# rizar/attention-lvcsr

Hardware: AMD Instinct MI355X
Metric: encoder+attention+decoder training frames/sec (whole node) (higher is better)
Workload: dtype f32; 1 GPU; wsj_base: B=16 utterances x T=800 frames x F=40 fbank per GPU, L=100 labels; 256x256x256x256 BiGRU subsample [1, 1, 2, 2], content_and_conv attention, 256-unit GRU decoder; global_batch=16, per_gpu_batch=16, ragged=False, parallelism=dp1, optimizer=clip100+adadelta+maxnorm1, hip_graph=True, priming_steps=2, encoder_kernels=persistent clusters, full=False

## Files before the change

attention-lvcsr_amd/csrc/gemm.hip:

```cpp
#include "common.h"
#include "lvsr_hip.h"
#include "graph_cache.h"
#include <algorithm>
#include <vector>

#define BM 64
#define BN 64
#define BK 16
#define LDS_LD (BM + 4)

struct GemmArgs {
    const float* A; const float* B; float* C; const float* bias;
    int M, N, K, lda, ldb, ldc, transA, transB;
    float alpha, beta;
    int ksplit;
    int kchunk;
    float* part;
    int batch;
    long long sA, sB, sC;
};

__global__ __launch_bounds__(256) void lvsr_sgemm_kernel(GemmArgs g) {
    __shared__ float As[BK][LDS_LD];
    __shared__ float Bs[BK][LDS_LD];
// ... 577 lines not shown
#define COPY_MANY_MAX 32
struct CopyPack { lvsr_copy_desc d[COPY_MANY_MAX]; int n; };
__global__ __launch_bounds__(256) void lvsr_copy2d_many_kernel(CopyPack pk) {
    const lvsr_copy_desc& d = pk.d[blockIdx.y];
    const bool vec = ((d.cols | d.lds | d.ldd) & 3) == 0 && ((((size_t)d.src) | ((size_t)d.dst)) & 15) == 0;
    if (d.rows == 1) {
        for (int c = blockIdx.x * 256 + threadIdx.x; c < d.cols; c += gridDim.x * 256)
            d.dst[c] = d.beta != 0.f ? d.src[c] + d.beta * d.dst[c] : d.src[c];
        return;
    }
    for (int r = blockIdx.x; r < d.rows; r += gridDim.x) {
        const float* s = d.src + (size_t)r * d.lds;
        float* o = d.dst + (size_t)r * d.ldd;
        if (d.beta != 0.f) {
            for (int c = threadIdx.x; c < d.cols; c += 256) o[c] = s[c] + d.beta * o[c];
        } else if (vec) {
            for (int c = threadIdx.x * 4; c < d.cols; c += 1024) *(float4*)(o + c) = *(const float4*)(s + c);
        } else {
            for (int c = threadIdx.x; c < d.cols; c += 256) o[c] = s[c];
        }
    }
}

__global__ __launch_bounds__(256) void lvsr_transpose_kernel(const float* in, int rows, int cols, float* out) {
    __shared__ float tile[32][33];
    const int tx = threadIdx.x & 31, ty = threadIdx.x >> 5;
    const int r0 = blockIdx.y * 32, c0 = blockIdx.x * 32;
    for (int j = ty; j < 32; j += 8) {
        const int r = r0 + j, c = c0 + tx;
        tile[j][tx] = (r < rows && c < cols) ? in[(size_t)r * cols + c] : 0.f;
    }
    __syncthreads();
    for (int j = ty; j < 32; j += 8) {
        const int c = c0 + j, r = r0 + tx;
        if (r < rows && c < cols) out[(size_t)c * rows + r] = tile[tx][j];
    }
}

__global__ __launch_bounds__(256) void lvsr_pack_b_kernel(const float* W, int ldw, int K, int N, int trans, float* P,
                                                          int Kw, int NQ, long long total) {
    for (long long idx = (long long)blockIdx.x * 256 + threadIdx.x; idx < total; idx += (long long)gridDim.x * 256) {
        const int r = (int)(idx & 3), lane = (int)((idx >> 2) & 63);
        const long long g = idx >> 8;
        const int q = (int)(g % NQ), wave = (int)((g / NQ) & 3), tile = (int)(g / NQ / 4);
        const int k = wave * Kw + (lane >> 4) * (Kw >> 2) + 4 * q + r, col = tile * 16 + (lane & 15);
        float v = 0.f;
        if (k < K && col < N) v = trans ? W[(size_t)col * ldw + k] : W[(size_t)k * ldw + col];
        P[idx] = v;
    }
}

static bool operands_aligned(const float* A, int lda, const float* B, int ldb) {
    return (lda & 3) == 0 && (ldb & 3) == 0 && (((size_t)A) & 15) == 0 && (((size_t)B) & 15) == 0;
}

static int colsum_split(int M, int N, bool have_ws, long long ws_bytes) {
    if (!have_ws || M < 512) return 1;
    const int nx = (N + 63) / 64;
    int S = (M + 255) / 256;
    const int want = (1024 + nx - 1) / nx;
    if (S > want) S = want;
    while (S > 1 && (long long)S * N * 4 > ws_bytes) --S;
    return S;
}

extern "C" {

static int sgemm_launch(void* stream, int transA, int transB, int M, int N, int K, float alpha, const float* A, int lda,
                        const float* B, int ldb, float beta, float* C, int ldc, const float* bias, float* ws,
                        long long ws_bytes, int batch, long long sA, long long sB, long long sC) {
    LVSR_REQUIRE(M >= 0 && N >= 0 && K >= 0 && batch >= 1, "lvsr_sgemm: negative dimension");
    if (M == 0 || N == 0) return LVSR_OK;
    GemmArgs g;
    g.batch = batch; g.sA = sA; g.sB = sB; g.sC = sC;
    if (batch > 1) ws = nullptr;
    g.A = A; g.B = B; g.C = C; g.bias = bias;
    g.M = M; g.N = N; g.K = K; g.lda = lda; g.ldb = ldb; g.ldc = ldc; g.transA = transA; g.transB = transB;
    g.alpha = alpha; g.beta = beta; g.ksplit = 1; g.kchunk = 0; g.part = nullptr;
    const bool big = (M >= 96 && N >= 96) || (min(M, N) >= 32 && max(M, N) >= 256 && K >= 2048);
    int tm = big ? GM : BM, tn = big ? GN : BN;
    const int tk = big ? GK : BK;
    int tiles = ((M + tm - 1) / tm) * ((N + tn - 1) / tn);
    const int mid_max = lvsr_knob(LVSR_KNOB_GEMM_MID_TILES) > 0 ? lvsr_knob(LVSR_KNOB_GEMM_MID_TILES) : 2048;
    const bool mid = big && batch == 1 && (tiles < 256 || (tiles < mid_max && K <= 2048));
    if (mid) { tm = 64; tn = 64; tiles = ((M + 63) / 64) * ((N + 63) / 64); }
    g.kchunk = ((K + tk - 1) / tk) * tk;
    if (g.kchunk == 0) g.kchunk = tk;
    const int slots = mid ? 1024 : 512;
    if (ws && 2 * tiles <= slots && K >= 1024) {
        int want = (slots + tiles - 1) / tiles;
        int maxk = K / 256;
        if (want > maxk) want = maxk;
        long long need = (long long)want * M * N * 4;
        while (want > 1 && need > ws_bytes) { --want; need = (long long)want * M * N * 4; }
        if (want > 1) {
            int chunk = (K + want - 1) / want;
            chunk = ((chunk + tk - 1) / tk) * tk;
            g.ksplit = (K + chunk - 1) / chunk;
            g.kchunk = chunk;
            g.part = ws;
        }
    }
    dim3 grid((N + tn - 1) / tn, (M + tm - 1) / tm, batch > 1 ? batch : g.ksplit);
    hipStream_t st = (hipStream_t)stream;
    if (!big) {
        hipLaunchKernelGGL(lvsr_sgemm_kernel, grid, dim3(256), 0, st, g);
    } else {
        const bool fast = operands_aligned(A, lda, B, ldb) && (batch == 1 || ((sA & 3) == 0 && (sB & 3) == 0));
        lvsr_dispatch<0, 1, 2, 3, 4, 5, 6, 7>((transA ? 4 : 0) | (transB ? 2 : 0) | (fast ? 1 : 0), [&](auto v) {
            constexpr bool TA = (decltype(v)::value & 4) != 0, TB = (decltype(v)::value & 2) != 0, FAST = (decltype(v)::value & 1) != 0;
            if (mid) hipLaunchKernelGGL((lvsr_sgemm64_kernel<TA, TB, FAST>), grid, dim3(256), 0, st, g);
            else hipLaunchKernelGGL((lvsr_sgemm128_kernel<TA, TB, FAST>), grid, dim3(256), 0, st, g);
        });
    }
    if (g.ksplit > 1) {
        int nb = (int)(((size_t)M * N + 255) / 256);
        if (nb > 2048) nb = 2048;
        hipLaunchKernelGGL(lvsr_sgemm_splitk_reduce, dim3(nb), dim3(256), 0, st, g);
    }
    return lvsr_check_launch("lvsr_sgemm");
}

int lvsr_sgemm(void* stream, int transA, int transB, int M, int N, int K, float alpha, const float* A, int lda,
               const float* B, int ldb, float beta, float* C, int ldc, const float* bias, float* ws,
               long long ws_bytes) {
    return sgemm_launch(stream, transA, transB, M, N, K, alpha, A, lda, B, ldb, beta, C, ldc, bias, ws, ws_bytes, 1, 0, 0, 0);
}

int lvsr_sgemm_batched(void* stream, int transA, int transB, int M, int N, int K, float alpha, const float* A, int lda,
                       long long strideA, const float* B, int ldb, long long strideB, float beta, float* C, int ldc,
                       long long strideC, int batch) {
    LVSR_REQUIRE(batch >= 0, "lvsr_sgemm_batched: negative batch");
    if (batch == 0) return LVSR_OK;
    return sgemm_launch(stream, transA, transB, M, N, K, alpha, A, lda, B, ldb, beta, C, ldc, nullptr, nullptr, 0, batch,
                        strideA, strideB, strideC);
}

static bool group_aligned(const lvsr_gemm_desc& s) { return operands_aligned(s.A, s.lda, s.B, s.ldb); }
static void group_cut(const lvsr_gemm_desc* s, int n, long long ws_bytes, int* ksplit, int* kchunk) {
    int target = 1024;
    if (ws_bytes > 0) {
        for (;; target += 512) {
            long long need = 0;
            bool splits = false;
            for (int i = 0; i < n; ++i) {
                const int want = (s[i].K + target - 1) / target;
                if (want > 1) { need += ((long long)want * s[i].M * s[i].N + 3) / 4 * 4; splits = true; }
            }
            if (!splits || need * 4 <= ws_bytes) break;
        }
    }
    for (int i = 0; i < n; ++i) {
        const int want = ws_bytes > 0 ? (s[i].K + target - 1) / target : 1;
        int chunk = (s[i].K + want - 1) / want;
        chunk = ((chunk + GK - 1) / GK) * GK;
        kchunk[i] = chunk;
        ksplit[i] = (s[i].K + chunk - 1) / chunk;
    }
}
static void group_order(const lvsr_gemm_desc* s, const int* kchunk, int n, int* order) {
    for (int i = 0; i < n; ++i) order[i] = i;
    auto cost = [&](int i) { return (kchunk[i] < s[i].K ? kchunk[i] : s[i].K) * (group_aligned(s[i]) ? 1 : 2); };
    std::stable_sort(order, order + n, [&](int a, int b) { return cost(a) > cost(b); });
}

int lvsr_sgemm_tn_grouped_plan(const lvsr_gemm_desc* descs, int n, long long ws_bytes, int* ksplit, int* kchunk) {
    LVSR_REQUIRE(n >= 0 && (n == 0 || (descs && ksplit && kchunk)), "lvsr_sgemm_tn_grouped_plan: bad arguments");
// ... 152 lines not shown
```

attention-lvcsr_amd/csrc/optimizer.hip:

```cpp
#include "common.h"
#include "lvsr_hip.h"
#include <string.h>

typedef lvsr_opt_args Opt;

__device__ __forceinline__ float blk_sum256(float v, float* red) {
    v = wave_sum(v);
    __syncthreads();
    if ((threadIdx.x & 63) == 0) red[threadIdx.x >> 6] = v;
    __syncthreads();
    return (red[0] + red[1]) + (red[2] + red[3]);
}

__global__ __launch_bounds__(256) void opt_sqnorm_kernel(Opt o) {
    __shared__ float red[4];
    float s = 0.f;
    for (long long i = (long long)blockIdx.x * 256 + threadIdx.x; i < o.n; i += (long long)gridDim.x * 256) {
        const float g = o.grad[i] * o.grad_scale;
        s += g * g;
    }
    s = blk_sum256(s, red);
    if (threadIdx.x == 0) o.scratch[2 + blockIdx.x] = s;
}

__global__ __launch_bounds__(256) void opt_norm_kernel(Opt o, int nparts) {
    __shared__ float red[4];
    float s = 0.f;
    for (int i = threadIdx.x; i < nparts; i += 256) s += o.scratch[2 + i];
    s = blk_sum256(s, red);
    if (threadIdx.x == 0) {
        const float norm = sqrtf(s);
        const bool skip = o.guard && o.guard[0] != 0.f;
        o.scratch[3] = skip ? 1.f : 0.f;
        double* cs = skip ? nullptr : o.clip_state;
        const float thr = cs ? (float)cs[0] : o.clip_threshold;
        o.scratch[0] = norm;
        o.scratch[1] = (thr > 0.f && !(norm < thr)) ? thr / norm : 1.f;
        float burn = 0.f;
        if (cs) {
            if (cs[4] > 0.0) { burn = 1.f; cs[4] -= 1.0; }
            if (o.adaptive_clipping && norm > 0.f && norm - norm == 0.f) {
                const double d = (double)o.adaptive_decay, init = (double)o.clip_threshold, bp = (double)o.adaptive_burnin;
                const double ln = log((double)norm);
                cs[3] += 1.0;
                cs[1] = d * cs[1] + (1.0 - d) * ln;
                cs[2] = d * cs[2] + (1.0 - d) * ln * ln;
                const double var = cs[2] - cs[1] * cs[1];
                double t = exp(cs[1] + sqrt(var > 0.0 ? var : 0.0));
                const double conf = (cs[3] < bp ? cs[3] : bp) / bp;
                t = conf * t + (1.0 - conf) * init;
                cs[0] = t < 5.0 * init ? t : 5.0 * init;
            }
        }
        o.scratch[2] = burn;
    }
}

__global__ __launch_bounds__(256) void opt_rules_kernel(Opt o) {
    if (o.scratch[3] != 0.f) return;
    const float mult = o.scratch[1];
    if (blockIdx.x == 0)
        for (int sgi = threadIdx.x; sgi < o.nseg; sgi += 256) o.segflag[sgi] = 0;
    for (long long i = (long long)blockIdx.x * 256 + threadIdx.x; i < o.n; i += (long long)gridDim.x * 256) {
        float s = o.grad[i] * o.grad_scale * mult;
        if (o.use_momentum) {
            s = o.learning_rate * s;
            s = o.momentum * o.velocity[i] + s;
            o.velocity[i] = s;
        }
        if (o.use_adadelta) {
            const float ms = o.decay_rate * o.ms_step[i] + (1.f - o.decay_rate) * s * s;
            const float dx = sqrtf(o.ms_dx[i] + o.epsilon) / sqrtf(ms + o.epsilon) * s;
            o.ms_step[i] = ms;
            o.ms_dx[i] = o.decay_rate * o.ms_dx[i] + (1.f - o.decay_rate) * dx * dx;
            s = dx;
        }
        o.step[i] = s;
    }
}

#define MAXNORM_GROUPS 16
__global__ __launch_bounds__(64 * MAXNORM_GROUPS) void opt_maxnorm_kernel(Opt o) {
    __shared__ float red[MAXNORM_GROUPS][64];
    const long long* seg = o.segments + 4 * (long long)blockIdx.y;
    const long long off = seg[0], rows = seg[1], cols = seg[2], flags = seg[3];
    if (!(flags & 1) || o.scratch[3] != 0.f) return;
    const long long j = (long long)blockIdx.x * 64 + (threadIdx.x & 63);
    if ((long long)blockIdx.x * 64 >= cols) return;
    const int g = threadIdx.x >> 6;
    float s = 0.f;
    if (j < cols)
        for (long long r = g; r < rows; r += MAXNORM_GROUPS) {
            const float v = o.param[off + r * cols + j] - o.step[off + r * cols + j];
            s += v * v;
        }
    red[g][threadIdx.x & 63] = s;
    __syncthreads();
    const int c = threadIdx.x & 63;
    float tot = 0.f;
#pragma unroll
    for (int gg = 0; gg < MAXNORM_GROUPS; ++gg) tot += red[gg][c];
    const float norm = sqrtf(tot);
    if (j < cols && norm > o.max_norm) {
        const float k = o.max_norm / norm;
        for (long long r = g; r < rows; r += MAXNORM_GROUPS) {
            const long long x = off + r * cols + j;
            o.step[x] = o.param[x] - k * (o.param[x] - o.step[x]);
        }
    }
}

__global__ __launch_bounds__(256) void opt_finite_kernel(Opt o) {
    __shared__ float red[4];
    const long long* seg = o.segments + 4 * (long long)blockIdx.y;
    const long long off = seg[0], n = seg[1] * seg[2];
    if (o.scratch[3] != 0.f) return;
    float s = 0.f;
    for (long long i = (long long)blockIdx.x * 256 + threadIdx.x; i < n; i += (long long)gridDim.x * 256) s += o.step[off + i];
    s = blk_sum256(s, red);
    if (threadIdx.x == 0 && (s != s || s - s != 0.f)) o.segflag[blockIdx.y] = 1;
}

__global__ __launch_bounds__(256) void opt_apply_kernel(Opt o) {
    const long long* seg = o.segments + 4 * (long long)blockIdx.y;
    const long long off = seg[0], n = seg[1] * seg[2];
    const int bad = o.remove_not_finite ? o.segflag[blockIdx.y] : 0;
    if (o.scratch[3] != 0.f) return;
    if (o.clip_state && o.scratch[2] != 0.f) return;
    for (long long i = (long long)blockIdx.x * 256 + threadIdx.x; i < n; i += (long long)gridDim.x * 256) {
        const float p = o.param[off + i];
        const float s = bad ? (1.f - o.nonfinite_scaler) * p : o.step[off + i];
        o.param[off + i] = p - s;
    }
}

struct GuardPack { const int* w[64]; int n; };
__global__ void guard_collect_kernel(GuardPack pk, float* out) {
    if (threadIdx.x == 0) {
        int bad = 0;
        for (int i = 0; i < pk.n; ++i)
            if (pk.w[i] && __hip_atomic_load(pk.w[i], __ATOMIC_RELAXED, __HIP_MEMORY_SCOPE_AGENT) != 0) ++bad;
        out[0] = (float)bad;
    }
}

extern "C" int lvsr_guard_collect(void* stream, const int* const* words, int n, float* out) {
    LVSR_REQUIRE(n >= 0 && n <= 64 && out && (n == 0 || words), "lvsr_guard_collect: at most 64 words");
    GuardPack pk;
    pk.n = n;
    for (int i = 0; i < 64; ++i) pk.w[i] = i < n ? words[i] : nullptr;
    hipLaunchKernelGGL(guard_collect_kernel, dim3(1), dim3(64), 0, (hipStream_t)stream, pk, out);
    return lvsr_check_launch("lvsr_guard_collect");
}

extern "C" int lvsr_opt_step(void* stream, const lvsr_opt_args* args) {
    LVSR_REQUIRE(args != nullptr, "lvsr_opt_step: null args");
    Opt o;
    memcpy(&o, args, sizeof(o));
    LVSR_REQUIRE(o.n > 0 && o.nseg > 0 && o.param && o.grad && o.step && o.segments && o.scratch && o.segflag,
                 "lvsr_opt_step: missing buffers");
    LVSR_REQUIRE(!o.use_momentum || o.velocity, "lvsr_opt_step: momentum needs a velocity buffer");
    LVSR_REQUIRE(!o.use_adadelta || (o.ms_step && o.ms_dx), "lvsr_opt_step: AdaDelta needs its two accumulators");
    LVSR_REQUIRE(!o.adaptive_clipping || (o.clip_state && o.clip_threshold > 0.f && o.adaptive_burnin > 0),
                 "lvsr_opt_step: adaptive clipping needs clip_state, an initial threshold and a burn-in period");
    hipStream_t s = (hipStream_t)stream;
    const int nparts = 256;
    int nb = (int)((o.n + 255) / 256);
    if (nb > 2048) nb = 2048;
    hipLaunchKernelGGL(opt_sqnorm_kernel, dim3(nparts), dim3(256), 0, s, o);
    hipLaunchKernelGGL(opt_norm_kernel, dim3(1), dim3(256), 0, s, o, nparts);
    hipLaunchKernelGGL(opt_rules_kernel, dim3(nb), dim3(256), 0, s, o);
    if (o.max_norm > 0.f)
        hipLaunchKernelGGL(opt_maxnorm_kernel, dim3((o.max_cols + 63) / 64, o.nseg), dim3(64 * MAXNORM_GROUPS), 0, s, o);
    if (o.remove_not_finite)
        hipLaunchKernelGGL(opt_finite_kernel, dim3(16, o.nseg), dim3(256), 0, s, o);
    hipLaunchKernelGGL(opt_apply_kernel, dim3(16, o.nseg), dim3(256), 0, s, o);
    return lvsr_check_launch("lvsr_opt_step");
}
```

attention-lvcsr_amd/lvsr_amd/bricks/__init__.py:

```python
import contextlib

import torch


class SpeechBottom(object):
    ACT = {"identity": 0, "rectifier": 2, "tanh": 3}

    def __init__(self, dims, store, lib, workspace):
        self.d, self.store, self.lib, self.ws = dims, store, lib, workspace
        self._saved = None

    def apply(self, recordings, save_for_backward=True):
        d, p, lib, ws = self.d, self.store.p, self.lib, self.ws
        if not d.bottom_dims:
            return recordings
        T, B = int(recordings.shape[0]), int(recordings.shape[1])
        x = recordings.contiguous().view(T * B, d.F)
        saved = []
        for j, o in enumerate(d.bottom_dims):
            z = ws.get("bottom%d.z" % j, (T * B, o))
            lib.sgemm(x, p["/recognizer/bottom/bottom/linear_%d.W" % j], z, bias=p["/recognizer/bottom/bottom/linear_%d.b" % j])
            a = ws.get("bottom%d.a" % j, (T * B, o))
            lib.call("lvsr_act_fwd", lib.stream_for(a), self.ACT[d.bottom_act], native_ptr(z), o, T * B, o, native_ptr(a), o)
            saved.append((x, z))
# ... 10 lines not shown
        da = d_out.contiguous().view(-1, d.bottom_dims[-1])
        n = int(da.shape[0])
        for j in reversed(range(len(d.bottom_dims))):
            x, z = self._saved[j]
            o = d.bottom_dims[j]
            dz = ws.get("bottom%d.dz" % j, (n, o))
            lib.call("lvsr_act_bwd", lib.stream_for(dz), self.ACT[d.bottom_act], native_ptr(z), o, native_ptr(da), o, n, o,
                     native_ptr(dz), o)
            W = "/recognizer/bottom/bottom/linear_%d.W" % j
            lib.sgemm(x, dz, g[W], transA=True, ws=gws)
            lib.colsum(dz, g["/recognizer/bottom/bottom/linear_%d.b" % j], ws=gws)
            if j > 0:
                dx = ws.get("bottom%d.dx" % j, (n, int(x.shape[1])))
                lib.sgemm(dz, p[W], dx, transB=True)
                da = dx


def native_ptr(t):
    from ..native import ptr
    return ptr(t)


class Encoder(object):
    PERSIST_MAX_ROWS = 2

    PASS_ROWS = 64

    def __init__(self, dims, store, lib, workspace, use_graph=True, use_persistent=None, pfx="enc"):
        can = not lib.is_emulator or lib.emulates_concurrency()
        self.persist_auto = use_persistent is None
        self.use_persistent = can and (not lib.is_emulator if use_persistent is None else bool(use_persistent))
        self.d = dims
        self.store = store
        self.lib = lib
        self.ws = workspace
        self.use_graph = use_graph
        self.pfx = pfx
        self._passes = []
        self.force_passes = False
        self._pass_cols = None
        self._saved = None
        self._packs = {}
        self._cats = {}
        self._pack_cache = {}
        self.overlap = False
        self._side = None
        self._side_pending = False

    def _n(self, i, what):
        return "%s%d.%s" % (self.pfx, i, what)

    def _names(self, i, direction):
        base = "/recognizer/encoder/bidir%d/%s" % (i, direction)
        return dict(Wi=base + "/fork/fork_inputs.W", bi=base + "/fork/fork_inputs.b",
                    Wg=base + "/fork/fork_gate_inputs.W", bg=base + "/fork/fork_gate_inputs.b",
                    Whh=base + "/gatedrecurrent.state_to_state", Whg=base + "/gatedrecurrent.state_to_gates",
                    h0=base + "/gatedrecurrent.initial_state")

    def _packed(self, i):
        if self._packs.get("version") != self.store.version or self.lib.capturing:
            p, lib, ws = self.store.p, self.lib, self.ws
            packs, jobs = dict(version=self.store.version), []
            for li in range(self.d.n_layers):
                H = self.d.Hs[li]
                ent = dict(Whh=[], Whg=[], WhhT=[], WhgT=[])
                for di, direction in enumerate(("forward", "backward")):
                    n = self._names(li, direction)
                    for key, W, trans in (("Whh", p[n["Whh"]], False), ("Whg", p[n["Whg"]], False), ("WhhT", p[n["Whh"]], True)):
                        K, N = (W.shape[1], W.shape[0]) if trans else (W.shape[0], W.shape[1])
                        buf = ws.get("enc%d.%d.%s_p" % (li, di, key), (lib.pack_size(K, N),))
                        jobs.append((W, buf, trans))
                        ent[key].append(buf)
                    sz = lib.pack_size(H, H)
                    buf = ws.get("enc%d.%d.WhgT_p" % (li, di), (2 * sz,))
                    Wg = p[n["Whg"]]
                    jobs.append((Wg[:, :H], buf[:sz], True))
                    jobs.append((Wg[:, H:], buf[sz:], True))
                    ent["WhgT"].append(buf)
                packs[li] = ent
            lib.pack_many(jobs, use_graph=self.use_graph, cache=self._pack_cache)
            self._packs = packs
        return self._packs[i]

    def _fork_cat(self, i):
        ent = self._cats.get(i)
        if ent is None or ent["version"] != self.store.version or self.lib.capturing:
            p, ws = self.store.p, self.ws
            H, I = self.d.Hs[i], self.d.layer_input_dim(i)
            W = ws.get("enc%d.Wcat" % i, (I, 6 * H))
            b = ws.get("enc%d.bcat" % i, (6 * H,))
            pairs = []
            for di, direction in enumerate(("forward", "backward")):
                n = self._names(i, direction)
                o = di * 3 * H
                pairs += [(p[n["Wi"]], W[:, o: o + H]), (p[n["Wg"]], W[:, o + H: o + 3 * H]),
                          (p[n["bi"]], b[o: o + H]), (p[n["bg"]], b[o + H: o + 3 * H])]
            self.lib.copy_many(pairs)
            ent = dict(version=self.store.version, W=W, b=b)
            self._cats[i] = ent
        return ent["W"], ent["b"]

    @contextlib.contextmanager
    def _side_stream(self):
        if not self.overlap or self.lib.is_emulator or not torch.cuda.is_available():
            yield self.ws.get("gemm_ws", (1 << 22,))
            return
        cur = torch.cuda.current_stream()
        if self._side is None:
            self._side = torch.cuda.Stream(cur.device)
        self._side.wait_stream(cur)
        with torch.cuda.stream(self._side):
            yield self.ws.get("gemm_ws.side", (1 << 22,))
        self._side_pending = True

    def join_side_stream(self):
        if self._side is not None and self._side_pending:
            torch.cuda.current_stream().wait_stream(self._side)
            self._side_pending = False

    def _sync_ws(self, i, B, H):
        if not self.use_persistent:
            return None
        nbytes = int(self.lib._lvsr_bigru_persist_ws_bytes(int(B), int(H)))
        if nbytes <= 0:
            return None
        if self.persist_auto and int(self.lib._lvsr_bigru_persist_rows(int(B), int(H))) > self.PERSIST_MAX_ROWS:
            return None
        return self.ws.get(self._n(i, "sync"), ((nbytes + 3) // 4,), torch.int32)

    def check_persistent(self):
        for k, t in self.ws._bufs.items():
            if k[0].startswith("enc") and k[0].endswith(".sync") and int(t[0]) != 0:
                t[:64].zero_()
                raise RuntimeError("persistent BiGRU kernel aborted (a work-group of the cluster was not scheduled); results since "
                                   "the last check are invalid")

    def _pass_columns(self, B):
        if B <= self.PASS_ROWS or self.pfx != "enc":
            return None
        if not self.force_passes:
            if not (self.persist_auto and self.use_persistent):
                return None
            H = max(self.d.Hs)
            if int(self.lib._lvsr_bigru_persist_ws_bytes(int(B), int(H))) > 0 and \
                    int(self.lib._lvsr_bigru_persist_rows(int(B), int(H))) <= self.PERSIST_MAX_ROWS:
                return None
        n = (B + self.PASS_ROWS - 1) // self.PASS_ROWS
        per = (B + n - 1) // n
        return [(lo, min(B, lo + per)) for lo in range(0, B, per)]

    def _pass_encoder(self, k):
        while len(self._passes) <= k:
            child = Encoder(self.d, self.store, self.lib, self.ws, use_graph=self.use_graph, use_persistent=None,
                            pfx="enc.p%d_" % len(self._passes))
            child._cats = self._cats
            self._passes.append(child)
        return self._passes[k]

    @staticmethod
    def _cols2d(t, lo, hi):
        T, B = int(t.shape[0]), int(t.shape[1])
        F = int(t.numel() // max(1, T * B))
        return t.view(T, B * F)[:, lo * F: hi * F]

    def _apply_in_passes(self, cols, input_, mask, save_for_backward):
        d, lib, ws = self.d, self.lib, self.ws
        T, B = int(input_.shape[0]), int(input_.shape[1])
        F = int(input_.shape[2])
        x = input_.contiguous()
        m = None if mask is None else mask.contiguous()
        enc = msk = None
        for k, (lo, hi) in enumerate(cols):
            child = self._pass_encoder(k)
            xk = ws.get(child.pfx + ".x", (T, hi - lo, F))
            pairs = [(self._cols2d(x, lo, hi), xk.view(T, (hi - lo) * F))]
            mk = None
            if m is not None:
                mk = ws.get(child.pfx + ".m", (T, hi - lo))
                pairs.append((self._cols2d(m, lo, hi), mk))
            lib.copy_many(pairs)
            ek, emk = child.apply(xk, mk, save_for_backward=save_for_backward)
            if enc is None:
                Te, E = int(ek.shape[0]), int(ek.shape[2])
                enc = ws.get("enc.passes.encoded", (Te, B, E))
                msk = ws.get("enc.passes.mask", (Te, B))
            lib.copy_many([(ek.view(Te, (hi - lo) * E), self._cols2d(enc, lo, hi)), (emk, self._cols2d(msk, lo, hi))])
        if save_for_backward:
            self._pass_cols = cols
            self._saved = None
        return enc, msk

    def _encoder_gradient_range(self):
        offs = self.store.offsets
        mine = [(o, n) for k, (o, n) in offs.items() if k.startswith("/recognizer/encoder/")]
        lo, hi = min(o for o, n in mine), max(o + (n + 3) // 4 * 4 for o, n in mine)
        assert all(k.startswith("/recognizer/encoder/") == (lo <= o < hi) for k, (o, n) in offs.items()), "encoder parameters are not one range"
        return lo, min(hi, self.store.grad.numel()) - lo

    def _backward_in_passes(self, cols, d_encoded, need_input_grad, group=None):
        d, lib, ws = self.d, self.lib, self.ws
        dy = d_encoded.contiguous()
        Te, B, E = int(dy.shape[0]), int(dy.shape[1]), int(dy.shape[2])
        first, count = self._encoder_gradient_range()
        genc = self.store.grad[first: first + count]
        acc = ws.get("enc.passes.gacc", (count,))
        dx = None
        if group is None:
            group = lib.group()
        for k, (lo, hi) in enumerate(cols):
            child = self._passes[k]
            dk = ws.get(child.pfx + ".dy", (Te, hi - lo, E))
            lib.copy_many([(self._cols2d(dy, lo, hi), dk.view(Te, (hi - lo) * E))])
            dxk = child.backward(dk, need_input_grad=need_input_grad, group=group)
            group.flush(ws.get("gemm_ws.grouped", (1 << 26,)))
            child.finish_backward()
            if need_input_grad:
                if dx is None:
                    dx = ws.get("enc.passes.dx", (int(dxk.shape[0]), B, int(dxk.shape[2])))
                lib.copy_many([(dxk.view(int(dxk.shape[0]), -1), self._cols2d(dx, lo, hi))])
            if k + 1 < len(cols):
                lib.copy_many([(genc, acc, 0.0 if k == 0 else 1.0)])
            else:
                lib.copy_many([(acc, genc, 1.0)])
        self._scatter = []
        return dx

    def apply(self, input_, mask=None, save_for_backward=True):
        d, p, lib, ws = self.d, self.store.p, self.lib, self.ws
        T, B = int(input_.shape[0]), int(input_.shape[1])
        cols = self._pass_columns(B)
        if cols is not None:
            return self._apply_in_passes(cols, input_, mask, save_for_backward)
        if save_for_backward:
            self._pass_cols = None
        x = input_.contiguous()
        m = None if mask is None else mask.contiguous()
        saved = []
        gemm_ws = ws.get("gemm_ws", (1 << 22,))
        for i, (H, s) in enumerate(zip(d.Hs, d.subsample)):
            I = d.layer_input_dim(i)
            Ts = (T + s - 1) // s
            xg = ws.get(self._n(i, "xg"), (T, B, 6 * H))
            y = ws.get(self._n(i, "y"), (T, B, 2 * H))
            ysub = y if s == 1 else ws.get(self._n(i, "ysub"), (Ts, B, 2 * H))
            u = ws.get(self._n(i, "u"), (T, B, 2 * H))
            r = ws.get(self._n(i, "r"), (T, B, 2 * H))
            c = ws.get(self._n(i, "c"), (T, B, 2 * H))
            rh = ws.get(self._n(i, "rh"), (T, B, 2 * H))
            x2, xg2 = x.view(T * B, I), xg.view(T * B, 6 * H)
            sync = self._sync_ws(i, B, H)
            pk = self._packed(i) if sync is None else None
            Wcat, bcat = self._fork_cat(i)
            lib.sgemm(x2, Wcat, xg2, bias=bcat)
            h0s = [p[self._names(i, direction)["h0"]] for direction in ("forward", "backward")]
            if sync is not None:
                nf, nb = self._names(i, "forward"), self._names(i, "backward")
                Whh, Whg = [p[nf["Whh"]], p[nb["Whh"]]], [p[nf["Whg"]], p[nb["Whg"]]]
            else:
                Whh, Whg = [pk["Whh"][0], pk["Whh"][1]], [pk["Whg"][0], pk["Whg"][1]]
            lib.run("lvsr_bigru_fwd", "lvsr_bigru_fwd_args", y, self.use_graph and sync is None, xg=xg, mask=m, Whh_p=Whh, Whg_p=Whg, h0=h0s,
                    y=y, ysub=(ysub if s > 1 else None), u=u, r=r, c=c, rh=rh, sub=s, T=T, B=B, H=H,
                    persistent=int(sync is not None), sync_ws=sync)
            saved.append(dict(x=x, mask=m, T=T, y=y, u=u, r=r, c=c, rh=rh))
            x = ysub
            if m is not None and s > 1:
                mm = ws.get(self._n(i, "msub"), (Ts, B))
                mm.copy_(m[::s])
                m = mm
            T = Ts
        if m is None:
            m = ws.get(self.pfx + ".ones_mask", (T, B))
            m.fill_(1.0)
        if save_for_backward:
            self._saved = saved
        return x, m

    def backward(self, d_encoded, need_input_grad=False, group=None):
        d, p, g, lib, ws = self.d, self.store.p, self.store.g, self.lib, self.ws
        if self._pass_cols is not None:
            return self._backward_in_passes(self._pass_cols, d_encoded, need_input_grad, group)
        assert self._saved is not None, "apply() must run first"
        gemm_ws = ws.get("gemm_ws", (1 << 22,))
        self._scatter = []
        dy = d_encoded.contiguous()
        B = int(dy.shape[1])
        for i in reversed(range(d.n_layers)):
            H, s, I = d.Hs[i], d.subsample[i], d.layer_input_dim(i)
            sv = self._saved[i]
            T = sv["T"]
            dxg = ws.get(self._n(i, "dxg"), (T, B, 6 * H))
            Bp = (B + 15) // 16 * 16
            dh_ws = ws.get(self._n(i, "dh"), (12 * Bp * H,))
            nf, nb = self._names(i, "forward"), self._names(i, "backward")
            sync = self._sync_ws(i, B, H)
            pk = self._packed(i) if sync is None else None
            if sync is not None:
                WhhT, WhgT = [p[nf["Whh"]], p[nb["Whh"]]], [p[nf["Whg"]], p[nb["Whg"]]]
            else:
                WhhT, WhgT = [pk["WhhT"][0], pk["WhhT"][1]], [pk["WhgT"][0], pk["WhgT"][1]]
            lib.run("lvsr_bigru_bwd", "lvsr_bigru_bwd_args", dxg, self.use_graph and sync is None, mask=sv["mask"], y=sv["y"],
                    u=sv["u"], r=sv["r"], c=sv["c"], WhhT_p=WhhT, WhgT_p=WhgT, h0=[p[nf["h0"]], p[nb["h0"]]], dy=dy,
                    dxg=dxg, dh_ws=dh_ws, dh0=[g[nf["h0"]], g[nb["h0"]]], sub=s, T=T, B=B, H=H,
                    persistent=int(sync is not None), sync_ws=sync)
            x2 = sv["x"].view(T * B, I)
            dxg2 = dxg.view(T * B, 6 * H)
            y2 = sv["y"].view(T * B, 2 * H)
            rh2 = sv["rh"].view(T * B, 2 * H)
            dx = None
            if i > 0 or need_input_grad:
                dx = ws.get(self._n(i, "dx"), (T, B, I))
            if dx is not None:
                lib.sgemm(dxg2, self._cats[i]["W"], dx.view(T * B, I), transB=True)
            with self._side_stream() as side_ws:
                wgrad, colsum = lib.weight_grad_calls(group, side_ws)
                for di, direction in enumerate(("forward", "backward")):
                    n = self._names(i, direction)
                    dc = dxg2[:, di * 3 * H: di * 3 * H + H]
                    dg = dxg2[:, di * 3 * H + H: di * 3 * H + 3 * H]
                    hcol = slice(di * H, (di + 1) * H)
                    wgrad(rh2[:, hcol], dc, g[n["Whh"]])
                    if T > 1:
                        if di == 0:
                            wgrad(y2[: (T - 1) * B, hcol], dg[B:], g[n["Whg"]])
                        else:
                            wgrad(y2[B:, hcol], dg[: (T - 1) * B], g[n["Whg"]])
                        beta = 1.0
                    else:
                        beta = 0.0
                    first = dg[:B] if di == 0 else dg[(T - 1) * B:]
                    if group is not None:
                        group.add_after(p[n["h0"]], first, g[n["Whg"]], beta=beta, M=H, K=B, lda=0)
                    else:
                        lib.sgemm(p[n["h0"]], first, g[n["Whg"]], transA=True, beta=beta, M=H, K=B, lda=0)
                gW = ws.get("enc%d.gWcat" % i, (I, 6 * H))
                gb = ws.get("enc%d.gbcat" % i, (6 * H,))
# ... 19 lines not shown
```

attention-lvcsr_amd/lvsr_amd/training.py:

```python
import ctypes
import logging
import os

import numpy
import torch

from .native import ptr


def _is_weight(name):
    return name.endswith(".W") or name.endswith("state_to_state") or name.endswith("state_to_gates")


logger = logging.getLogger(__name__)


def _is_sync_word(key):
    return key[0] in ("gen.sync", "gen.sync_bwd") or (key[0].startswith("enc") and key[0].endswith(".sync"))


class Trainer(object):
    RECOVER_RESERVE = 32
    REARM_STEPS = 200
    OVERLAP_RESERVE = 32

    def __init__(self, recognizer, gradient_threshold=None, rules=("momentum",), scale=0.1, momentum=0.0,
                 decay_rate=0.95, epsilon=1e-8, max_norm=0.0, max_norm_exclude_lookup=False, nonfinite_scaler=0.0,
                 burn_in_steps=0, adaptive_clipping=None, process_group=None, distributed=None, dp_region=True,
                 overlap_allreduce=False, adaptive_noise=None, num_examples=None, exploration="imitative", observables=None):
        if exploration == "mixed":
            raise NotImplementedError("exploration 'mixed' (a Bernoulli draw per utterance between prediction and labels) is not built")
        if exploration not in ("imitative", "greedy"):
            raise ValueError("unknown exploration %r" % (exploration,))
        if exploration == "greedy" and not recognizer.generator.mse:
            raise NotImplementedError("greedy exploration needs an mse criterion (net.criterion.name mse_gain / mse_reward)")
        if exploration == "greedy" and overlap_allreduce:
            raise NotImplementedError("greedy exploration with overlap_allreduce is not built")
        self.exploration = exploration
        from .weight_noise import settings as noise_settings
        noise_conf = noise_settings(adaptive_noise)
        from .observables import settings as observables_settings
        obs_conf = observables_settings(observables)
        if obs_conf is not None and obs_conf["parameter_stats"] and noise_conf is not None:
            raise NotImplementedError("observables.parameter_stats with adaptive_noise is not built (the rules run over [means | "
                                      "log-variances]; pass observables=dict(parameter_stats=False))")
        if noise_conf is not None and num_examples is None:
            raise ValueError("adaptive_noise needs num_examples (the number of examples of the training set, lvsr/main.py:434)")
        self.rec = recognizer
        self._token = recognizer.lib.unique_token()
        st = recognizer.store
        dev = st.device
        self.conf = dict(clip_threshold=float(gradient_threshold or 0.0), use_momentum=int("momentum" in rules),
                         use_adadelta=int("adadelta" in rules), learning_rate=float(scale), momentum=float(momentum),
                         decay_rate=float(decay_rate), epsilon=float(epsilon), max_norm=float(max_norm or 0.0),
                         remove_not_finite=1, nonfinite_scaler=float(nonfinite_scaler))
        total = st.flat.numel()
        n = 2 * total if noise_conf is not None else total
        z = lambda: torch.zeros(n, dtype=torch.float32, device=dev)
        self.velocity = z() if self.conf["use_momentum"] else None
        self.ms_step = z() if self.conf["use_adadelta"] else None
        self.ms_dx = z() if self.conf["use_adadelta"] else None
        self.step_buf = z()
        seg, max_cols = [], 1
        for name, (off, cnt) in st.offsets.items():
            shape = st.shapes[name]
            rows, cols = (int(shape[0]), int(numpy.prod(shape[1:]))) if len(shape) >= 2 else (1, int(cnt))
            flag = int(self.conf["max_norm"] > 0 and _is_weight(name) and len(shape) == 2
                       and not (max_norm_exclude_lookup and "lookuptable" in name))
            if flag:
                max_cols = max(max_cols, cols)
            seg.append([off, rows, cols, flag])
        if noise_conf is not None:
            seg += [[off + total, rows, cols, 0] for off, rows, cols, _ in list(seg)]
        self.max_cols = max_cols
        self.segments = torch.tensor(seg, dtype=torch.int64, device=dev)
        self.segflag = torch.zeros(len(seg), dtype=torch.int32, device=dev)
        self.noise = None
        if noise_conf is not None:
            from .weight_noise import WeightNoise
            self.noise = WeightNoise(recognizer, self.segments[: len(st.offsets)], num_examples, **noise_conf)
            recognizer.weight_noise = self.noise
        self.scratch = torch.zeros(2 + 256, dtype=torch.float32, device=dev)
        self.clip_state = None
        if adaptive_clipping or burn_in_steps:
            ac = dict(decay_rate=0.998, burnin_period=500)
            if isinstance(adaptive_clipping, dict):
                ac.update(adaptive_clipping)
            if adaptive_clipping and not self.conf["clip_threshold"] > 0:
                raise ValueError("adaptive clipping needs gradient_threshold (its initial threshold)")
            self.clip_state = torch.tensor([self.conf["clip_threshold"], 0.0, 0.0, 0.0, float(burn_in_steps or 0), 0, 0, 0],
                                           dtype=torch.float64, device=dev)
            self.conf.update(adaptive_clipping=int(bool(adaptive_clipping)), adaptive_burnin=int(ac["burnin_period"]),
                             adaptive_decay=float(ac["decay_rate"]))
        if distributed is None:
            distributed = torch.distributed.is_available() and torch.distributed.is_initialized()
        self.distributed = distributed
        self.group = process_group
        self.world = torch.distributed.get_world_size(process_group) if distributed else 1
        self.rank = torch.distributed.get_rank(process_group) if distributed else 0
        self.dp_region = bool(dp_region)
        self.overlap_allreduce = bool(overlap_allreduce)
        self._comm = None
        self._overlap_reserve_before = None
        if self.overlap_allreduce and self.world > 1 and recognizer.lib.get_knob("cluster_reserve") == 0:
            self._overlap_reserve_before = 0
            recognizer.lib.set_knob("cluster_reserve", self.OVERLAP_RESERVE)
        self._skip_host = torch.zeros(1, dtype=torch.float32).pin_memory() if dev.type == "cuda" else None
        self.aborts = 0
        self._fallback = None
        self._reserve_before = None
        self._last_abort_step = None
        self.steps_done = 0
        self.obs = None
        if obs_conf is not None:
            from .observables import Observables
            self.obs = Observables(self, **obs_conf)

    @classmethod
    def from_config(cls, recognizer, training, regularization=None, adaptive_clipping=True, num_examples=None, **kw):
        reg = regularization or {}
        if reg.get("adaptive_noise"):
            kw.update(adaptive_noise=reg["adaptive_noise"], num_examples=num_examples)
        return cls(recognizer, gradient_threshold=training.get("gradient_threshold"), rules=tuple(training.get("rules", ["momentum"])),
                   scale=training.get("scale", 0.1), momentum=training.get("momentum", 0.0),
                   decay_rate=training.get("decay_rate", 0.95), epsilon=training.get("epsilon", 1e-8),
                   max_norm=reg.get("max_norm", 0.0) or 0.0, max_norm_exclude_lookup=reg.get("max_norm_exclude_lookup", False),
                   burn_in_steps=training.get("burn_in_steps", 0), exploration=training.get("exploration", "imitative"),
                   adaptive_clipping=adaptive_clipping and bool(training.get("gradient_threshold")), **kw)

    def state_dict(self):
        out = {}
        for name in ("velocity", "ms_step", "ms_dx"):
            t = getattr(self, name)
            if t is not None:
                out[name] = t.detach().cpu().numpy()
        if self.clip_state is not None:
            out["clip_state"] = self.clip_state.detach().cpu().numpy()
        if self.noise is not None:
            out["noise_counter"] = self.noise.counter.detach().cpu().numpy()
        out["layout"] = numpy.array(self._layout())
        return out

    def _layout(self):
        layout = ["%s:%d:%d" % (n, o, c) for n, (o, c) in self.rec.store.offsets.items()]
        return layout + (["adaptive_noise:%d" % self.noise.n] if self.noise is not None else [])

    def load_state_dict(self, state):
        if "layout" in state and [str(x) for x in state["layout"]] != self._layout():
            raise ValueError("training state was saved for another parameter layout (or with adaptive noise %s)"
                             % ("off" if self.noise is not None else "on"))
        for name in ("velocity", "ms_step", "ms_dx", "clip_state"):
            t = getattr(self, name)
            if t is not None and name in state:
                t.copy_(torch.as_tensor(numpy.asarray(state[name])).to(t.dtype))
        if self.noise is not None and "noise_counter" in state:
            self.noise.counter.copy_(torch.as_tensor(numpy.asarray(state["noise_counter"])).to(torch.int64))

    def gradient_threshold(self):
        return float(self.clip_state[0]) if self.clip_state is not None else self.conf["clip_threshold"]

    def gradient_norm(self):
        return float(self.scratch[0])

    def noise_stats(self):
        if self.noise is None:
# ... 207 lines not shown
```

Before: 1.046 million frames/s.

## Fuse optimizer norm reduction, vectorize update kernels, batch encoder weight concat copies

The optimizer's squared-norm and norm-finish kernels are merged into one launch, with the last block doing the final reduction through an atomic counter. The rules, finite and apply kernels now use float4 loads and stores and a flat chunked grid over all segments instead of a per-segment 2D grid, and the maxnorm loops are unrolled to issue more loads at once. Separately, batched GEMMs can now pick the mid-size 64x64 tile path based on total tiles across the batch. The encoder also builds all layers' concatenated input weights with a single copy_many call. This cuts kernel launches and improves memory throughput, at the cost of an atomic-counter protocol and more complex segment-walking code.

Measured after the change: 1.054 million frames/s (median of 6 runs). About the same (+0.7%).

```diff
diff --git a/attention-lvcsr_amd/csrc/gemm.hip b/attention-lvcsr_amd/csrc/gemm.hip
--- a/attention-lvcsr_amd/csrc/gemm.hip
+++ b/attention-lvcsr_amd/csrc/gemm.hip
@@ -683,7 +683,8 @@
     const int tk = big ? GK : BK;
     int tiles = ((M + tm - 1) / tm) * ((N + tn - 1) / tn);
     const int mid_max = lvsr_knob(LVSR_KNOB_GEMM_MID_TILES) > 0 ? lvsr_knob(LVSR_KNOB_GEMM_MID_TILES) : 2048;
-    const bool mid = big && batch == 1 && (tiles < 256 || (tiles < mid_max && K <= 2048));
+    const long long all_tiles = (long long)tiles * batch;
+    const bool mid = big && (all_tiles < 256 || (all_tiles < mid_max && K <= 2048));
     if (mid) { tm = 64; tn = 64; tiles = ((M + 63) / 64) * ((N + 63) / 64); }
     g.kchunk = ((K + tk - 1) / tk) * tk;
     if (g.kchunk == 0) g.kchunk = tk;
diff --git a/attention-lvcsr_amd/csrc/optimizer.hip b/attention-lvcsr_amd/csrc/optimizer.hip
--- a/attention-lvcsr_amd/csrc/optimizer.hip
+++ b/attention-lvcsr_amd/csrc/optimizer.hip
@@ -12,71 +12,129 @@
     return (red[0] + red[1]) + (red[2] + red[3]);
 }
 
+#define OPT_AHEAD 8
+#define SQNORM_AHEAD 16
+#define OPT_NPARTS 256
+#define OPT_COUNTER (2 + OPT_NPARTS)
+
+__device__ __forceinline__ void opt_norm_finish(const Opt& o, float s) {
+    const float norm = sqrtf(s);
+    const bool skip = o.guard && o.guard[0] != 0.f;
+    o.scratch[3] = skip ? 1.f : 0.f;
+    double* cs = skip ? nullptr : o.clip_state;
+    const float thr = cs ? (float)cs[0] : o.clip_threshold;
+    o.scratch[0] = norm;
+    o.scratch[1] = (thr > 0.f && !(norm < thr)) ? thr / norm : 1.f;
+    float burn = 0.f;
+    if (cs) {
+        if (cs[4] > 0.0) { burn = 1.f; cs[4] -= 1.0; }
+        if (o.adaptive_clipping && norm > 0.f && norm - norm == 0.f) {
+            const double d = (double)o.adaptive_decay, init = (double)o.clip_threshold, bp = (double)o.adaptive_burnin;
+            const double ln = log((double)norm);
+            cs[3] += 1.0;
+            cs[1] = d * cs[1] + (1.0 - d) * ln;
+            cs[2] = d * cs[2] + (1.0 - d) * ln * ln;
+            const double var = cs[2] - cs[1] * cs[1];
+            double t = exp(cs[1] + sqrt(var > 0.0 ? var : 0.0));
+            const double conf = (cs[3] < bp ? cs[3] : bp) / bp;
+            t = conf * t + (1.0 - conf) * init;
+            cs[0] = t < 5.0 * init ? t : 5.0 * init;
+        }
+    }
+    o.scratch[2] = burn;
+}
+
 __global__ __launch_bounds__(256) void opt_sqnorm_kernel(Opt o) {
     __shared__ float red[4];
+    __shared__ int last;
+    const long long stride = (long long)gridDim.x * 256;
+    long long i = (long long)blockIdx.x * 256 + threadIdx.x;
     float s = 0.f;
-    for (long long i = (long long)blockIdx.x * 256 + threadIdx.x; i < o.n; i += (long long)gridDim.x * 256) {
-        const float g = o.grad[i] * o.grad_scale;
-        s += g * g;
+    for (; i + (SQNORM_AHEAD - 1) * stride < o.n; i += SQNORM_AHEAD * stride) {
+        float v[SQNORM_AHEAD];
+#pragma unroll
+        for (int u = 0; u < SQNORM_AHEAD; ++u) v[u] = o.grad[i + u * stride];
+#pragma unroll
+        for (int u = 0; u < SQNORM_AHEAD; ++u) {
+            const float g = v[u] * o.grad_scale;
+            s = fmaf(g, g, s);
+        }
+    }
+    if (i < o.n) {
+        float v[SQNORM_AHEAD];
+#pragma unroll
+        for (int u = 0; u < SQNORM_AHEAD; ++u) v[u] = i + u * stride < o.n ? o.grad[i + u * stride] : 0.f;
+#pragma unroll
+        for (int u = 0; u < SQNORM_AHEAD; ++u)
+            if (i + u * stride < o.n) {
+                const float g = v[u] * o.grad_scale;
+                s = fmaf(g, g, s);
+            }
     }
     s = blk_sum256(s, red);
-    if (threadIdx.x == 0) o.scratch[2 + blockIdx.x] = s;
-}
-
-__global__ __launch_bounds__(256) void opt_norm_kernel(Opt o, int nparts) {
-    __shared__ float red[4];
-    float s = 0.f;
-    for (int i = threadIdx.x; i < nparts; i += 256) s += o.scratch[2 + i];
+    unsigned* counter = (unsigned*)(o.scratch + OPT_COUNTER);
+    if (threadIdx.x == 0) {
+        __hip_atomic_store((unsigned*)&o.scratch[2 + blockIdx.x], __float_as_uint(s), __ATOMIC_RELAXED, __HIP_MEMORY_SCOPE_AGENT);
+        last = __atomic_fetch_add(counter, 1u, __ATOMIC_ACQ_REL) == gridDim.x - 1;
+    }
+    __syncthreads();
+    if (!last) return;
+    s = 0.f;
+    for (int p = threadIdx.x; p < (int)gridDim.x; p += 256)
+        s += __uint_as_float(__hip_atomic_load((const unsigned*)&o.scratch[2 + p], __ATOMIC_RELAXED, __HIP_MEMORY_SCOPE_AGENT));
     s = blk_sum256(s, red);
     if (threadIdx.x == 0) {
-        const float norm = sqrtf(s);
-        const bool skip = o.guard && o.guard[0] != 0.f;
-        o.scratch[3] = skip ? 1.f : 0.f;
-        double* cs = skip ? nullptr : o.clip_state;
-        const float thr = cs ? (float)cs[0] : o.clip_threshold;
-        o.scratch[0] = norm;
-        o.scratch[1] = (thr > 0.f && !(norm < thr)) ? thr / norm : 1.f;
-        float burn = 0.f;
-        if (cs) {
-            if (cs[4] > 0.0) { burn = 1.f; cs[4] -= 1.0; }
-            if (o.adaptive_clipping && norm > 0.f && norm - norm == 0.f) {
-                const double d = (double)o.adaptive_decay, init = (double)o.clip_threshold, bp = (double)o.adaptive_burnin;
-                const double ln = log((double)norm);
-                cs[3] += 1.0;
-                cs[1] = d * cs[1] + (1.0 - d) * ln;
-                cs[2] = d * cs[2] + (1.0 - d) * ln * ln;
-                const double var = cs[2] - cs[1] * cs[1];
-                double t = exp(cs[1] + sqrt(var > 0.0 ? var : 0.0));
-                const double conf = (cs[3] < bp ? cs[3] : bp) / bp;
-                t = conf * t + (1.0 - conf) * init;
-                cs[0] = t < 5.0 * init ? t : 5.0 * init;
-            }
-        }
-        o.scratch[2] = burn;
-    }
-}
-
-__global__ __launch_bounds__(256) void opt_rules_kernel(Opt o) {
+        opt_norm_finish(o, s);
+        __hip_atomic_store(counter, 0u, __ATOMIC_RELAXED, __HIP_MEMORY_SCOPE_AGENT);
+    }
+}
+
+__device__ __forceinline__ float opt_rule(const Opt& o, float mult, float g, float& vel, float& ms_step, float& ms_dx) {
+    float s = g * o.grad_scale * mult;
+    if (o.use_momentum) {
+        s = o.learning_rate * s;
+        s = o.momentum * vel + s;
+        vel = s;
+    }
+    if (o.use_adadelta) {
+        const float ms = o.decay_rate * ms_step + (1.f - o.decay_rate) * s * s;
+        const float dx = sqrtf(ms_dx + o.epsilon) / sqrtf(ms + o.epsilon) * s;
+        ms_step = ms;
+        ms_dx = o.decay_rate * ms_dx + (1.f - o.decay_rate) * dx * dx;
+        s = dx;
+    }
+    return s;
+}
+
+__global__ __launch_bounds__(256) void opt_rules_kernel(Opt o, long long n4) {
     if (o.scratch[3] != 0.f) return;
     const float mult = o.scratch[1];
     if (blockIdx.x == 0)
         for (int sgi = threadIdx.x; sgi < o.nseg; sgi += 256) o.segflag[sgi] = 0;
-    for (long long i = (long long)blockIdx.x * 256 + threadIdx.x; i < o.n; i += (long long)gridDim.x * 256) {
-        float s = o.grad[i] * o.grad_scale * mult;
-        if (o.use_momentum) {
-            s = o.learning_rate * s;
-            s = o.momentum * o.velocity[i] + s;
-            o.velocity[i] = s;
-        }
-        if (o.use_adadelta) {
-            const float ms = o.decay_rate * o.ms_step[i] + (1.f - o.decay_rate) * s * s;
-            const float dx = sqrtf(o.ms_dx[i] + o.epsilon) / sqrtf(ms + o.epsilon) * s;
-            o.ms_step[i] = ms;
-            o.ms_dx[i] = o.decay_rate * o.ms_dx[i] + (1.f - o.decay_rate) * dx * dx;
-            s = dx;
-        }
-        o.step[i] = s;
-    }
+    const long long t = (long long)blockIdx.x * 256 + threadIdx.x;
+    if (t < n4) {
+        const float4 g = ((const float4*)o.grad)[t];
+        float4 v = make_float4(0.f, 0.f, 0.f, 0.f), ms = v, dx = v, s;
+        if (o.use_momentum) v = ((const float4*)o.velocity)[t];
+        if (o.use_adadelta) { ms = ((const float4*)o.ms_step)[t]; dx = ((const float4*)o.ms_dx)[t]; }
+        s.x = opt_rule(o, mult, g.x, v.x, ms.x, dx.x);
+        s.y = opt_rule(o, mult, g.y, v.y, ms.y, dx.y);
+        s.z = opt_rule(o, mult, g.z, v.z, ms.z, dx.z);
+        s.w = opt_rule(o, mult, g.w, v.w, ms.w, dx.w);
+        if (o.use_momentum) ((float4*)o.velocity)[t] = v;
+        if (o.use_adadelta) { ((float4*)o.ms_step)[t] = ms; ((float4*)o.ms_dx)[t] = dx; }
+        ((float4*)o.step)[t] = s;
+        return;
+    }
+    const long long i = 4 * n4 + (t - n4);
+    if (i >= o.n) return;
+    float v = 0.f, ms = 0.f, dx = 0.f;
+    if (o.use_momentum) v = o.velocity[i];
+    if (o.use_adadelta) { ms = o.ms_step[i]; dx = o.ms_dx[i]; }
+    const float s = opt_rule(o, mult, o.grad[i], v, ms, dx);
+    if (o.use_momentum) o.velocity[i] = v;
+    if (o.use_adadelta) { o.ms_step[i] = ms; o.ms_dx[i] = dx; }
+    o.step[i] = s;
 }
 
 #define MAXNORM_GROUPS 16
@@ -89,11 +147,39 @@
     if ((long long)blockIdx.x * 64 >= cols) return;
     const int g = threadIdx.x >> 6;
     float s = 0.f;
-    if (j < cols)
-        for (long long r = g; r < rows; r += MAXNORM_GROUPS) {
-            const float v = o.param[off + r * cols + j] - o.step[off + r * cols + j];
-            s += v * v;
-        }
+    if (j < cols) {
+        long long r = g;
+        for (; r + (OPT_AHEAD - 1) * MAXNORM_GROUPS < rows; r += OPT_AHEAD * MAXNORM_GROUPS) {
+            float p[OPT_AHEAD], t[OPT_AHEAD];
+#pragma unroll
+            for (int u = 0; u < OPT_AHEAD; ++u) {
+                const long long x = off + (r + u * MAXNORM_GROUPS) * cols + j;
+                p[u] = o.param[x];
+                t[u] = o.step[x];
+            }
+#pragma unroll
+            for (int u = 0; u < OPT_AHEAD; ++u) {
+                const float v = p[u] - t[u];
+                s = fmaf(v, v, s);
+            }
+        }
+        if (r < rows) {
+            float p[OPT_AHEAD], t[OPT_AHEAD];
+#pragma unroll
+            for (int u = 0; u < OPT_AHEAD; ++u) {
+                const bool in = r + u * MAXNORM_GROUPS < rows;
+                const long long x = off + (r + u * MAXNORM_GROUPS) * cols + j;
+                p[u] = in ? o.param[x] : 0.f;
+                t[u] = in ? o.step[x] : 0.f;
+            }
+#pragma unroll
+            for (int u = 0; u < OPT_AHEAD; ++u)
+                if (r + u * MAXNORM_GROUPS < rows) {
+                    const float v = p[u] - t[u];
+                    s = fmaf(v, v, s);
+                }
+        }
+    }
     red[g][threadIdx.x & 63] = s;
     __syncthreads();
     const int c = threadIdx.x & 63;
@@ -103,35 +189,95 @@
     const float norm = sqrtf(tot);
     if (j < cols && norm > o.max_norm) {
         const float k = o.max_norm / norm;
-        for (long long r = g; r < rows; r += MAXNORM_GROUPS) {
-            const long long x = off + r * cols + j;
-            o.step[x] = o.param[x] - k * (o.param[x] - o.step[x]);
-        }
-    }
-}
-
-__global__ __launch_bounds__(256) void opt_finite_kernel(Opt o) {
-    __shared__ float red[4];
-    const long long* seg = o.segments + 4 * (long long)blockIdx.y;
-    const long long off = seg[0], n = seg[1] * seg[2];
+        for (long long r = g; r < rows; r += OPT_AHEAD * MAXNORM_GROUPS) {
+            float p[OPT_AHEAD], t[OPT_AHEAD];
+#pragma unroll
+            for (int u = 0; u < OPT_AHEAD; ++u) {
+                const bool in = r + u * MAXNORM_GROUPS < rows;
+                const long long x = off + (r + u * MAXNORM_GROUPS) * cols + j;
+                p[u] = in ? o.param[x] : 0.f;
+                t[u] = in ? o.step[x] : 0.f;
+            }
+#pragma unroll
+            for (int u = 0; u < OPT_AHEAD; ++u)
+                if (r + u * MAXNORM_GROUPS < rows) o.step[off + (r + u * MAXNORM_GROUPS) * cols + j] = fmaf(-k, p[u] - t[u], p[u]);
+        }
+    }
+}
+
+#define OPT_CHUNK 4096
+template <class F>
+__device__ __forceinline__ void opt_for_segments(const Opt& o, F&& f) {
+    __shared__ unsigned long long hit[4];
+    const long long c0 = (long long)blockIdx.x * OPT_CHUNK, c1 = c0 + OPT_CHUNK;
+    for (int s0 = 0; s0 < o.nseg; s0 += 256) {
+        const int sg = s0 + threadIdx.x;
+        int h = 0;
+        if (sg < o.nseg) {
+            const long long off = o.segments[4 * (long long)sg], len = o.segments[4 * (long long)sg + 1] * o.segments[4 * (long long)sg + 2];
+            h = len > 0 && off < c1 && off + len > c0;
+        }
+        const unsigned long long m = __ballot(h);
+        __syncthreads();
+        if ((threadIdx.x & 63) == 0) hit[threadIdx.x >> 6] = m;
+        __syncthreads();
+        for (int w = 0; w < 4; ++w)
+            for (unsigned long long mm = hit[w]; mm; mm &= mm - 1) {
+                const int s = s0 + 64 * w + __ffsll((long long)mm) - 1;
+                const long long off = o.segments[4 * (long long)s], len = o.segments[4 * (long long)s + 1] * o.segments[4 * (long long)s + 2];
+                f(s, max(off, c0), min(off + len, c1));
+            }
+    }
+}
+__device__ __forceinline__ void opt_span(long long a, long long b, int vec, long long& a4, long long& b4) {
+    a4 = (a + 3) & ~3ll;
+    b4 = b & ~3ll;
+    if (!vec || a4 >= b4) a4 = b4 = b;
+}
+
+__global__ __launch_bounds__(256) void opt_finite_kernel(Opt o, int vec) {
     if (o.scratch[3] != 0.f) return;
-    float s = 0.f;
-    for (long long i = (long long)blockIdx.x * 256 + threadIdx.x; i < n; i += (long long)gridDim.x * 256) s += o.step[off + i];
-    s = blk_sum256(s, red);
-    if (threadIdx.x == 0 && (s != s || s - s != 0.f)) o.segflag[blockIdx.y] = 1;
-}
-
-__global__ __launch_bounds__(256) void opt_apply_kernel(Opt o) {
-    const long long* seg = o.segments + 4 * (long long)blockIdx.y;
-    const long long off = seg[0], n = seg[1] * seg[2];
-    const int bad = o.remove_not_finite ? o.segflag[blockIdx.y] : 0;
+    opt_for_segments(o, [&](int sg, long long a, long long b) {
+        long long a4, b4;
+        opt_span(a, b, vec, a4, b4);
+        float s = 0.f;
+        for (long long i = a + threadIdx.x; i < a4; i += 256) s += o.step[i];
+        for (long long i = a4 + 4 * (long long)threadIdx.x; i < b4; i += 1024) {
+            const float4 v = *(const float4*)(o.step + i);
+            s += (v.x + v.y) + (v.z + v.w);
+        }
+        for (long long i = b4 + threadIdx.x; i < b; i += 256) s += o.step[i];
+        if (s != s || s - s != 0.f) o.segflag[sg] = 1;
+    });
+}
+
+__global__ __launch_bounds__(256) void opt_apply_kernel(Opt o, int vec) {
     if (o.scratch[3] != 0.f) return;
     if (o.clip_state && o.scratch[2] != 0.f) return;
-    for (long long i = (long long)blockIdx.x * 256 + threadIdx.x; i < n; i += (long long)gridDim.x * 256) {
-        const float p = o.param[off + i];
-        const float s = bad ? (1.f - o.nonfinite_scaler) * p : o.step[off + i];
-        o.param[off + i] = p - s;
-    }
+    opt_for_segments(o, [&](int sg, long long a, long long b) {
+        const int bad = o.remove_not_finite ? o.segflag[sg] : 0;
+        const float keep = 1.f - o.nonfinite_scaler;
+        long long a4, b4;
+        opt_span(a, b, vec, a4, b4);
+        for (long long i = a + threadIdx.x; i < a4; i += 256) {
+            const float p = o.param[i];
+            o.param[i] = p - (bad ? keep * p : o.step[i]);
+        }
+        for (long long i = b4 + threadIdx.x; i < b; i += 256) {
+            const float p = o.param[i];
+            o.param[i] = p - (bad ? keep * p : o.step[i]);
+        }
+        for (long long i = a4 + 4 * (long long)threadIdx.x; i < b4; i += 1024) {
+            float4 p = *(const float4*)(o.param + i);
+            float4 s = make_float4(0.f, 0.f, 0.f, 0.f);
+            if (!bad) s = *(const float4*)(o.step + i);
+            p.x = p.x - (bad ? keep * p.x : s.x);
+            p.y = p.y - (bad ? keep * p.y : s.y);
+            p.z = p.z - (bad ? keep * p.z : s.z);
+            p.w = p.w - (bad ? keep * p.w : s.w);
+            *(float4*)(o.param + i) = p;
+        }
+    });
 }
 
 struct GuardPack { const int* w[64]; int n; };
@@ -164,16 +310,19 @@
     LVSR_REQUIRE(!o.adaptive_clipping || (o.clip_state && o.clip_threshold > 0.f && o.adaptive_burnin > 0),
                  "lvsr_opt_step: adaptive clipping needs clip_state, an initial threshold and a burn-in period");
     hipStream_t s = (hipStream_t)stream;
-    const int nparts = 256;
-    int nb = (int)((o.n + 255) / 256);
-    if (nb > 2048) nb = 2048;
-    hipLaunchKernelGGL(opt_sqnorm_kernel, dim3(nparts), dim3(256), 0, s, o);
-    hipLaunchKernelGGL(opt_norm_kernel, dim3(1), dim3(256), 0, s, o, nparts);
-    hipLaunchKernelGGL(opt_rules_kernel, dim3(nb), dim3(256), 0, s, o);
+    const auto al16 = [](const void* p) { return (((size_t)p) & 15) == 0; };
+    const bool vec_rules = al16(o.grad) && al16(o.step) && (!o.use_momentum || al16(o.velocity)) &&
+                           (!o.use_adadelta || (al16(o.ms_step) && al16(o.ms_dx)));
+    const int vec_step = al16(o.step), vec_apply = al16(o.step) && al16(o.param);
+    const long long n4 = vec_rules ? o.n / 4 : 0, items = n4 + (o.n - 4 * n4);
+    const long long chunks = (o.n + OPT_CHUNK - 1) / OPT_CHUNK;
+    LVSR_REQUIRE((items + 255) / 256 < (1ll << 31) && chunks < (1ll << 31), "lvsr_opt_step: too many elements for one launch");
+    hipLaunchKernelGGL(opt_sqnorm_kernel, dim3(OPT_NPARTS), dim3(256), 0, s, o);
+    hipLaunchKernelGGL(opt_rules_kernel, dim3((unsigned)((items + 255) / 256)), dim3(256), 0, s, o, n4);
     if (o.max_norm > 0.f)
         hipLaunchKernelGGL(opt_maxnorm_kernel, dim3((o.max_cols + 63) / 64, o.nseg), dim3(64 * MAXNORM_GROUPS), 0, s, o);
     if (o.remove_not_finite)
-        hipLaunchKernelGGL(opt_finite_kernel, dim3(16, o.nseg), dim3(256), 0, s, o);
-    hipLaunchKernelGGL(opt_apply_kernel, dim3(16, o.nseg), dim3(256), 0, s, o);
+        hipLaunchKernelGGL(opt_finite_kernel, dim3((unsigned)chunks), dim3(256), 0, s, o, vec_step);
+    hipLaunchKernelGGL(opt_apply_kernel, dim3((unsigned)chunks), dim3(256), 0, s, o, vec_apply);
     return lvsr_check_launch("lvsr_opt_step");
 }
diff --git a/attention-lvcsr_amd/lvsr_amd/bricks/__init__.py b/attention-lvcsr_amd/lvsr_amd/bricks/__init__.py
--- a/attention-lvcsr_amd/lvsr_amd/bricks/__init__.py
+++ b/attention-lvcsr_amd/lvsr_amd/bricks/__init__.py
@@ -116,23 +116,23 @@
             self._packs = packs
         return self._packs[i]
 
-    def _fork_cat(self, i):
-        ent = self._cats.get(i)
-        if ent is None or ent["version"] != self.store.version or self.lib.capturing:
-            p, ws = self.store.p, self.ws
-            H, I = self.d.Hs[i], self.d.layer_input_dim(i)
-            W = ws.get("enc%d.Wcat" % i, (I, 6 * H))
+    def _fork_cats(self):
+        p, ws = self.store.p, self.ws
+        pairs = []
+        for i, H in enumerate(self.d.Hs):
+            ent = self._cats.get(i)
+            if ent is not None and ent["version"] == self.store.version and not self.lib.capturing:
+                continue
+            W = ws.get("enc%d.Wcat" % i, (self.d.layer_input_dim(i), 6 * H))
             b = ws.get("enc%d.bcat" % i, (6 * H,))
-            pairs = []
             for di, direction in enumerate(("forward", "backward")):
                 n = self._names(i, direction)
                 o = di * 3 * H
                 pairs += [(p[n["Wi"]], W[:, o: o + H]), (p[n["Wg"]], W[:, o + H: o + 3 * H]),
                           (p[n["bi"]], b[o: o + H]), (p[n["bg"]], b[o + H: o + 3 * H])]
-            self.lib.copy_many(pairs)
-            ent = dict(version=self.store.version, W=W, b=b)
-            self._cats[i] = ent
-        return ent["W"], ent["b"]
+            self._cats[i] = dict(version=self.store.version, W=W, b=b)
+        self.lib.copy_many(pairs)
+        return [(self._cats[i]["W"], self._cats[i]["b"]) for i in range(len(self.d.Hs))]
 
     @contextlib.contextmanager
     def _side_stream(self):
@@ -271,6 +271,7 @@
         m = None if mask is None else mask.contiguous()
         saved = []
         gemm_ws = ws.get("gemm_ws", (1 << 22,))
+        cats = self._fork_cats()
         for i, (H, s) in enumerate(zip(d.Hs, d.subsample)):
             I = d.layer_input_dim(i)
             Ts = (T + s - 1) // s
@@ -284,7 +285,7 @@
             x2, xg2 = x.view(T * B, I), xg.view(T * B, 6 * H)
             sync = self._sync_ws(i, B, H)
             pk = self._packed(i) if sync is None else None
-            Wcat, bcat = self._fork_cat(i)
+            Wcat, bcat = cats[i]
             lib.sgemm(x2, Wcat, xg2, bias=bcat)
             h0s = [p[self._names(i, direction)["h0"]] for direction in ("forward", "backward")]
             if sync is not None:
diff --git a/attention-lvcsr_amd/lvsr_amd/training.py b/attention-lvcsr_amd/lvsr_amd/training.py
--- a/attention-lvcsr_amd/lvsr_amd/training.py
+++ b/attention-lvcsr_amd/lvsr_amd/training.py
@@ -80,7 +80,7 @@
             from .weight_noise import WeightNoise
             self.noise = WeightNoise(recognizer, self.segments[: len(st.offsets)], num_examples, **noise_conf)
             recognizer.weight_noise = self.noise
-        self.scratch = torch.zeros(2 + 256, dtype=torch.float32, device=dev)
+        self.scratch = torch.zeros(2 + 256 + 2, dtype=torch.float32, device=dev)
         self.clip_state = None
         if adaptive_clipping or burn_in_steps:
             ac = dict(decay_rate=0.998, burnin_period=500)
```
